# geometryxyz/mental-poker

Measured on AMD Instinct MI355X. Metric: shuffle proofs/sec (prove+verify), higher is better.
Workload: dtype u32 limbs (256-bit Montgomery: 9x29-bit lazy base field, 8x32 scalar field); 1 GPU; pairs: 52-card deck, m=2 n=26, stark curve, shuffle_and_remask + verify_shuffle; rccl_world=1, fixed_base_window_bits=21, unit_counted=prove+verify pairs, streams=1, aggregate_keys=1, transcript_lanes=1, prover_streams=1, pipeline_depth=0, validated_once=False, full=False

## Files before the change

mental-poker_amd/csrc/engine_core.hpp:

```cpp
#pragma once
#include "engine_base.hpp"
#include "kernels_bucket.hpp"
#include "kernels_decompress.hpp"
#include "kernels_sigma.hpp"
#include "kernels_open.hpp"
#include "kernels_deal.hpp"
#include "serialize_host.hpp"
#include "setup_host.hpp"

namespace mp {

static const uint32_t FCHUNK = 8;
static const uint32_t VCHUNK = 64;
static const uint32_t NORM_CHUNK = 64;
static const uint32_t BUCKET_MIN = 2048;
static const uint32_t BUCKET_MIN_SMALL_BATCH = 512;

struct PhaseDev {
  DevBuf<Term> recode, tables, fterms, vterms, cterms, cterms2, cterms0;
  DevBuf<Job> fjobs, vjobs, cjobs, cjobs2, cjobs0;
  DevBuf<BJob> bjobs;
  DevBuf<Term> bterms;
  DevBuf<BTermPos> bpos;
  DevBuf<Job> wcjobs;
// ... 34 lines not shown
    b_bits = ph.b_bits;
    n_recode = (uint32_t)ph.recode.size();
    n_tables = (uint32_t)ph.tables.size();
    n_f = (uint32_t)ph.fjobs.size();
    n_v = (uint32_t)ph.vjobs.size();
    n_c = (uint32_t)ph.cjobs.size();
    n_tslots = ph.n_tslots;
    n_dslots = ph.n_dslots;
    normalize = ph.normalize;
  }
};

struct Workspace {
  uint32_t fw = 8;
  uint32_t Bpad = 0;
  uint32_t nS = 0, nP = 0, nJ = 0, nD = 0, nT = 0, nwin = 0, stage_words = 0;
  DevBuf<uint32_t> S, P, J, T, NS, NS2, stage, seed, direct;
  DevBuf<uint32_t> W;
  DevBuf<int8_t> D;
  DevBuf<int16_t> D16;
  uint32_t d8_bytes = 0;
  DevBuf<uint32_t> bk_sorted, bk_park, bk_counter, bk_timing, bk_quarters;
  DevBuf<uint16_t> bk_offs;
  void ensure_bucket(uint32_t nslots, uint32_t kpad_max, uint32_t bits, uint32_t xw, rt::Stream s) {
    bk_sorted.alloc((size_t)nslots * kpad_max, s, false);
    bk_park.alloc((size_t)nslots * bk_buckets(bits) * xw, s, false);
    bk_counter.alloc(8, s);
  }
  DevBuf<int32_t> status;
  uint32_t cap = 0;
  void ensure(uint32_t B, uint32_t nS_, uint32_t nP_, uint32_t nJ_, uint32_t nD_, uint32_t nT_, uint32_t nwin_,
              uint32_t stage_words_, rt::Stream s, uint32_t d8_bytes_ = 0) {
    const uint32_t need = (B + 63u) & ~63u;
    const bool grow = !(need <= cap && nS_ <= nS && nP_ <= nP && nJ_ <= nJ && nD_ <= nD && nT_ <= nT && stage_words_ <= stage_words &&
                        d8_bytes_ <= d8_bytes);
    if (grow) {
      cap = std::max(cap, need);
      nS = std::max(nS, nS_); nP = std::max(nP, nP_); nJ = std::max(nJ, nJ_); nD = std::max(nD, nD_); nT = std::max(nT, nT_);
      nwin = nwin_;
      stage_words = std::max(stage_words, stage_words_);
      S.n = P.n = J.n = T.n = NS.n = stage.n = seed.n = direct.n = 0;
      D.n = 0;
      D16.n = 0;
      d8_bytes = std::max(d8_bytes, d8_bytes_);
      D16.alloc((size_t)std::max(d8_bytes, 4u) * cap, s);
      status.n = 0;
      S.alloc((size_t)nS * cap * 8, s);
      P.alloc((size_t)nP * cap * 2 * fw, s);
      J.alloc((size_t)nJ * cap * 3 * fw, s);
      D.alloc((size_t)std::max(nD, 1u) * nwin * cap, s);
      T.alloc((size_t)std::max(nT, 1u) * VB_ENTRIES * cap * 2 * fw, s);
      size_t norm_max = std::max((size_t)nT * 8, (size_t)nJ) * cap;
      NS.alloc(norm_max * fw, s);
      stage.alloc((size_t)stage_words * cap, s);
      seed.alloc((size_t)8 * cap, s);
      direct.alloc((size_t)2 * cap, s);
      status.alloc(cap, s);
      Bpad = need;
      return;
    }
    if (Bpad != need) {
      Bpad = need;
      rt::dzero(J.p, (size_t)nJ * Bpad * 3 * fw * sizeof(uint32_t), s);
    }
  }
};

template <class C>
struct Table : mp_table {
// ... 202 lines not shown
  DevBuf<uint32_t> vflag;
  uint32_t* flag_word(bool vlane, rt::Stream s) {
    if (!vflag.n) vflag.alloc(2, s);
    rt::dzero(vflag.p + (vlane ? 1 : 0), 4, s);
    return vflag.p + (vlane ? 1 : 0);
  }
  bool read_flag(bool vlane) {
    uint32_t flag = 0;
    rt::d2h(&flag, vflag.p + (vlane ? 1 : 0), 4, ctx->stream);
    rt::stream_sync(ctx->stream);
    return flag != 0;
  }
  uint32_t nwin = 0;
  FbGeom fbg{8, 32, 255};
  uint32_t init_seed[8];
  DevBuf<uint8_t> io_a, io_b, io_c, io_d, io_e, io_f;
  DevBuf<int32_t> io_status;

  static bool wire_point_host(const uint8_t* p, Aff<C>& out) {
    alignas(8) uint8_t tmp[G_::PB];
    memcpy(tmp, p, G_::PB);
    return wire_to_aff<C>(tmp, out);
  }

  void build_plans(PlanSet* set, bool keyed) {
    rt::Stream s = ctx->stream;
    for (int k = 0; k < N_PLANS; ++k) {
      PlanSet& q = set[k];
      const PlanParams& pp = pprm[k];
      const uint32_t bmin = (bucket_min && k == 3) ? std::min(bucket_min, BUCKET_MIN_SMALL_BATCH) : bucket_min;
// ... 76 lines not shown
      fe_pack<F>(bases[i].x, &flat[i * G_::PW]);
      fe_pack<F>(bases[i].y, &flat[i * G_::PW + G_::FW]);
    }
    fbpts.upload(flat, s);
    build_fixed_tables(fb.count());

    build_plans(ps, false);
    {
      Blake2sState st;
      blake2s_init(st);
      uint32_t mblk[16] = {0};
      memcpy(mblk, "Shuffle Proof", 13);
      blake2s_compress(st, mblk, 13, true);
      memcpy(init_seed, st.h, 32);
    }
    rt::stream_sync(s);
    return MP_OK;
  }

  void normalize_flat(const uint32_t* src, uint32_t* dst, uint32_t* scratch, size_t count) {
    if (!count) return;
    const uint32_t ch = cur_norm_chunk;
    NormArgs a{src, dst, scratch, (uint32_t)count, (uint32_t)((count + ch - 1) / ch), ch};
    MP_RUN(k_normalize, C, a.nthreads, 1, a);
  }

  void build_narrow_tables(const uint32_t* pts, uint32_t nb, const FbGeom& gh, uint32_t h2, uint32_t* out) {
    rt::Stream s = ctx->stream;
    DevBuf<uint32_t> WJ, W, EJ, scratch;
    const size_t nwinpts = (size_t)nb * gh.windows, nent = nwinpts * gh.entries;
// ... 62 lines not shown
      const uint32_t kc = (uint32_t)std::min(slice, K - k0);
      build_narrow_tables(pts.p + k0 * G_::PW, kc, g8, 8u, ks.FB.p + k0 * per_key);
    }
    rt::stream_sync(s);
    return MP_OK;
  }
  DevBuf<uint32_t> ks_keys_main, ks_keys_vlane;
  const uint8_t* gather_keys(uint32_t B, const mp_keyset* ks, const uint32_t* kidx, int32_t* status, bool vlane = false) {
    DevBuf<uint32_t>& ks_keys = vlane ? ks_keys_vlane : ks_keys_main;
    ks_keys.alloc((size_t)B * (G_::PB / 4), ctx->stream, false);
    GatherKeysArgs ga{ks->wire.p, kidx, ks_keys.p, status, (uint32_t)ks->K};
    MP_RUN(k_gather_keys, C, B, G_::PB / 4, ga);
    return reinterpret_cast<const uint8_t*>(ks_keys.p);
  }

  uint32_t stage_words_needed() const {
    const size_t tb = G_::PB + 1;
    size_t bytes = (size_t)(3 + n + 1 + 4 * N) * tb + 16 + 32;
    bytes = std::max(bytes, (size_t)(1 + 6 * m) * tb + 32);
    return (uint32_t)(bytes / 4 + 4);
  }

  void reserve(size_t B) override { reserve_for(B, false); }
  void reserve_for(size_t B, bool keyed) { reserve_ws(ws, B, keyed); }
  void reserve_ws(Workspace& ws, size_t B, bool keyed) {
    if (keyed) ensure_keyed();
    PlanSet& q = pick((uint32_t)B, keyed);
    uint32_t nS = std::max(q.pplan.lay.nS, q.vplan.lay.nS), nP = std::max(q.pplan.lay.nP, q.vplan.lay.nP);
    uint32_t nJ = std::max(q.pplan.nJ, q.vplan.nJ), nD = std::max(q.vph.n_dslots, q.vmph.n_dslots),
             nT = std::max(q.vph.n_tslots, q.vmph.n_tslots);
    uint32_t d8 = std::max(q.vph.b_dig_bytes, q.vmph.b_dig_bytes);
    for (int i = 0; i < 6; ++i) {
      nD = std::max(nD, q.pph[i].n_dslots);
      nT = std::max(nT, q.pph[i].n_tslots);
      d8 = std::max(d8, q.pph[i].b_dig_bytes);
    }
    if (keyed) {
      nD = std::max(nD, key_d_first + N);
      nT = std::max(nT, key_t_first + nwin);
    }
    ws.fw = G_::FW;
    ws.ensure((uint32_t)B, nS, nP, nJ, nD, nT, nwin, stage_words_needed(), ctx->stream, d8);
    if (&ws == &this->ws && overlap_max && B <= overlap_max) ws.NS2.alloc((size_t)m * ws.Bpad * G_::FW, ctx->stream, false);
  }

  enum : uint32_t { PH_RECODE = 1, PH_TABLES = 2, PH_MSM = 4, PH_NORM = 8, PH_ALL = 15 };
  void run_phase(PhaseDev& ph, Workspace& w, uint32_t B, uint32_t parts = PH_ALL, uint32_t norm_only = NO_SLOT, uint32_t norm_skip = NO_SLOT,
                 uint32_t* scratch = nullptr) {
    if (!scratch) scratch = w.NS.p;
    if (parts & PH_TABLES) run_tables(ph, w, B, scratch);
    if (parts & PH_RECODE) run_recode(ph, w, B);
    if (parts & PH_MSM) run_msms(ph, w, B);
    if (parts & PH_NORM) run_normalize(ph, w, B, norm_only, norm_skip, scratch);
  }
#ifdef MP_EXP_QUAD_MAX
  uint32_t quad_max_lanes = MP_EXP_QUAD_MAX;
#else
// ... 204 lines not shown
    }
  }

  FsStatementArgs statement_args(Workspace& w, uint32_t p_deck, uint32_t p_shuf, uint32_t p_cA, uint32_t s_x, uint32_t p_pk = NO_SLOT) {
    FsStatementArgs a{};
    a.f = FsDev{w.stage.p, w.seed.p, w.Bpad};
    a.S = w.S.p;
    a.P = w.P.p;
    a.fbpts = fbpts.p;
    memcpy(a.init_seed, init_seed, 32);
    a.m = m; a.n = n; a.N = N;
    a.p_deck = p_deck; a.p_shuf = p_shuf; a.p_cA = p_cA; a.s_x = s_x;
    a.p_pk = p_pk;
    a.W = nullptr;
    a.w_deck = a.w_shuf = NO_SLOT;
    return a;
  }
  FsqGeom fsq_geom(uint32_t B) const {
    uint32_t lpp = 64;
    while (lpp > 4 && (uint64_t)B * lpp > 65536u) lpp >>= 1;
    return FsqGeom{lpp, B};
  }
  static uint32_t fsq_waves(const FsqGeom& g) { return (g.B + 64u / g.lpp - 1) / (64u / g.lpp); }
  bool fs_quad(uint32_t B) const { return fs_lanes == 4 || (fs_lanes == 0 && B <= FSQ_MAX_BATCH); }
  void run_fs_round1(const FsStatementArgs& a, uint32_t B) {
    if (fs_quad(B)) {
      FsqStatementArgs q{a, fsq_geom(B)};
      MP_WAVE_RUN(k_fsq_round1, C, fsq_waves(q.g), 0, q);
    } else {
      MP_RUN(k_fs_round1, C, B, 1, a);
    }
  }
  void run_fs_round(const FsRoundArgs& a, uint32_t B) {
    if (fs_quad(B)) {
      FsqRoundArgs q{a, fsq_geom(B)};
      MP_WAVE_RUN(k_fsq_round, C, fsq_waves(q.g), 0, q);
    } else {
      MP_RUN(k_fs_round, C, B, 1, a);
    }
  }
  void run_verify_fs(const VerifyFsArgs& a, uint32_t B) {
    if (fs_quad(B)) {
      FsqVerifyArgs q{a, fsq_geom(B)};
      MP_WAVE_RUN(k_fsq_verify, C, fsq_waves(q.g), 0, q);
    } else {
      MP_RUN(k_verify_fs, C, B, 1, a);
    }
  }
  uint32_t* wire_words(Workspace& w, uint32_t B, uint32_t decks) {
    const int plan = plan_of(B);
    if (plan != 1 && plan != 3 && plan != 5) return nullptr;
    w.W.alloc((size_t)decks * 2 * N * (G_::PB / 4) * w.Bpad, ctx->stream, false);
    return w.W.p;
  }

  void prove_init(const ProveInitArgs& ia, uint32_t B) {
    if (B <= PROVE_INIT_WAVE_MAX)
// ... 628 lines not shown
            if (j == 0) var(ChainTerm{l.mvar + l.deck + i, g, 1, NO_SLOT, G}, l.deck + i, g);
            else if (j < L) var(ChainTerm{l.mvar + l.deck + i, j * G + g, 1, l.mvar + l.shuf + i, G}, l.deck + i, j * G + g);
            else var(ChainTerm{l.mvar + l.shuf + i, (L - 1) * G + g, 1, NO_SLOT, G}, l.shuf + i, (L - 1) * G + g);
          }
      for (uint32_t j = 0; j < L * G; ++j)
        for (uint32_t slot = l.cA; slot < l.pk; ++slot) var(ChainTerm{l.mvar + slot, j, 1, NO_SLOT, 1}, slot, j);
      if (keyed)
        for (uint32_t g = 0; g < G; ++g) var(ChainTerm{l.mvar + l.pk, g, L, NO_SLOT, G}, l.pk, g);
    });
    chain.dtile_src.upload(chain.tile_src, ctx->stream);
  }
  size_t chain_lane_bytes(uint32_t, bool keyed) override {
    if (keyed) ensure_keyed();
    const VerifyLay& l = (keyed ? psk : ps)[0].vplan.lay;
    const size_t fwb = (size_t)G_::FW * 4, nJ = 4 + bk_windows(R::BITS, 8);
    return (size_t)l.nS * 32 + (size_t)l.nP * 2 * fwb + nJ * 3 * fwb + nwin + (size_t)VB_ENTRIES * 2 * fwb + nJ * fwb + (size_t)stage_words_needed() * 4 + 32 + 8 + 4 + 8;
  }
  size_t chain_lanes_held() const override { return cws.cap; }
  uint32_t chain_group_size(size_t T, uint32_t L, bool keyed) const override { return T < 0x7FFFFFFFu ? chain_group_of((uint32_t)T, L, keyed) : 1u; }
  void size_equations(const ChainPlan& p, uint32_t T, uint32_t L) {
    const uint32_t Tpad = (T + 63u) & ~63u;
    chain_cw.alloc((size_t)L * Tpad * 8, ctx->stream, false);
    chain_cs.alloc((size_t)(p.K + p.nfix) * Tpad * 8, ctx->stream);
    chain_d8.alloc((size_t)p.dev.b_dig_bytes * Tpad, ctx->stream);
  }
  struct EquationArgs {
    uint32_t T, L;
    bool vlane;
    const char* too_many;
    uint32_t pk, G;
    uint32_t* flag;
// ... 28 lines not shown
      gbad[e.vlane ? 1 : 0].alloc(T, s, false);
      gb = gbad[e.vlane ? 1 : 0].p;
    }
    ChainVerdictArgs va{w.J.p, w.direct.p, w.status.p, e.flag ? e.flag : flag_word(e.vlane, s), gb, w.Bpad, T, e.L, 0u, w.P.p, e.pk, e.G, e.status, nullptr};
    run_chain_verdict(va);
  }
  void verify_chain_dev(size_t T_, uint32_t L, const uint8_t* decks, const uint8_t* proofs, int32_t* status, const uint8_t* keys) override {
    const uint32_t T = (uint32_t)T_, B = T * L;
    const bool keyed = keys != nullptr;
    const uint32_t G = chain_group_of(T, L, keyed), Tq = T / G, Lq = L * G;
    build_chain_plan(L, keyed, G);
    PlanSet& q = (keyed ? psk : ps)[0];
    const VerifyLay& l = q.vplan.lay;
    Workspace& w = cws;
    w.fw = G_::FW;
    w.ensure(B, l.nS, l.nP, std::max(chain.nJ, 8u), 0, 0, nwin, stage_words_needed(), ctx->stream, 0);
    const VArgs cv{B, decks, decks + (size_t)T * 2 * N * G_::PB, proofs, status, keys, nullptr, nullptr};
    load_verify_inputs(w, q, cv, false, false);
    run_transcripts(w, q, B, keyed, true, false);
    run_verify_scalars(w, q, B, true);
    size_equations(chain, Tq, Lq);
    run_chain_weights(w, (Tq + 63u) & ~63u, Tq, Lq);
    const EquationArgs e{Tq, Lq, false, "chain verification: too many tables for one launch", keyed ? l.pk : NO_SLOT, G, nullptr, nullptr, status};
    run_equations(w, chain, e, true, [&](uint32_t* run) {
      ChainTileArgs ta{w.P.p, run, chain.dtile_src.p, w.Bpad, Tq, chain.K};
      if ((uint64_t)Tq * chain.K >= ((uint64_t)1 << 32)) throw std::runtime_error("chain verification: too many tables for one launch");
      MP_RUN(k_chain_tile, C, Tq * chain.K, 1, ta);
    });
    if (!read_flag(false)) return;
    refine_groups(cv, gbad[0].p, false, Tq, Lq, false, false, 0, 0, false);
  }
// ... 68 lines not shown
      for (uint32_t j = 0; j < L; ++j)
        for (uint32_t slot = 0; slot < per; ++slot)
          term(ChainTerm{l.mvar + slot, j, 1, NO_SLOT, 1}, bk_tile ? j * per + slot : (slot | (j << 20)));
    });
    return *fresh;
  }
  void verify_group_pass(const VArgs& v, uint32_t L, bool vlane, uint32_t* host_flag, uint32_t* gbad_out) {
    const uint32_t B = v.B, T = B / L;
    const bool keyed = v.keys != nullptr || v.kset != nullptr;
    ChainPlan& gplan = build_group_plan(L, keyed);
    PlanSet& q = (keyed ? psk : ps)[0];
    const VerifyLay& l = q.vplan.lay;
    rt::Stream s = ctx->stream;
    Workspace& w = vlane ? gws : ws;
    w.fw = G_::FW;
    w.ensure(B, l.nS, l.nP, std::max(gplan.nJ, 8u), 0, 0, nwin, stage_words_needed(), s, 0);
    load_verify_inputs(w, q, v, vlane, false);
    run_transcripts(w, q, B, keyed, true, false);
    size_equations(gplan, T, L);
    {
      SideGuard wguard{ctx, false};
      {
        SideFork on_side(ctx);
        run_chain_weights(w, (T + 63u) & ~63u, T, L);
        rt::event_record(ctx->ev_tab, ctx->side);
      }
      run_verify_scalars(w, q, B, true);
      rt::stream_wait(s, ctx->ev_tab);
      wguard.joined = true;
    }
    const uint32_t per = l.pk + (keyed ? 1u : 0u);
// ... 149 lines not shown
          pb.end();
        }
        pb.normalize(l.A, nb);
      } else {
        for (uint32_t i = 0; i < nb; ++i) {
          pb.begin(l.chk + i);
          pb.var(l.z, l.g + i);
          pb.var(l.negc, l.a + i);
          pb.var(l.minus_one, l.A + i);
          pb.end();
        }
      }
    }
    ad.dev.upload(ad.ph, s);
    ad.w.fw = G_::FW;
    ad.w.ensure(B, 6, 3 * nb, next_partial, ad.ph.n_dslots, ad.ph.n_tslots, nwin, (3 * nb * (G_::PB + 1) + 32) / 4 + 4, s);
    Workspace& w = ad.w;
    DevBuf<uint8_t> dg, da, dx, dfs, dseed, dpf;
    DevBuf<int32_t> dst;
    dg.alloc((size_t)B * nb * G_::PB, s, false); da.alloc((size_t)B * nb * G_::PB, s, false); dfs.alloc((size_t)B * 32, s, false);
    dpf.alloc((size_t)B * psz, s, false);
    rt::h2d(dg.p, bases, (size_t)B * nb * G_::PB, s);
    rt::h2d(da.p, publics, (size_t)B * nb * G_::PB, s);
    rt::h2d(dfs.p, fs_init, (size_t)B * 32, s);
    rt::dzero(w.status.p, (size_t)w.Bpad * 4, s);
    LoadPointsArgs lg{dg.p, w.P.p, w.status.p, w.Bpad, nb, l.g};
    MP_RUN(k_load_points, C, B, nb, lg);
    LoadPointsArgs la{da.p, w.P.p, w.status.p, w.Bpad, nb, l.a};
    MP_RUN(k_load_points, C, B, nb, la);
    check_subgroup(w, B, l.g, 2 * nb);
    const FsDev f{w.stage.p, w.seed.p, w.Bpad};
// ... 82 lines not shown
        op.nD = std::max(op.nD, ph->n_dslots);
        op.nT = std::max(op.nT, ph->n_tslots);
      }
      op.vdev.upload(op.vph, s);
      op.rdev1.upload(op.rph1, s);
      op.rdev2.upload(op.rph2, s);
      Blake2sState st;
      blake2s_init(st);
      uint32_t mblk[16] = {0};
      memcpy(mblk, "Reveal Proof", 12);
      blake2s_compress(st, mblk, 12, true);
      memcpy(op.fs_seed, st.h, 32);
      op.ready = true;
    }
    op.w.fw = G_::FW;
    op.w.ensure(B, 6, 6, op.nJ, op.nD, op.nT, nwin, (6 * (G_::PB + 1) + 32) / 4 + 4, s);
    op.fs.alloc((size_t)op.w.cap * 32, s, false);
    rt::dzero(op.w.status.p, (size_t)op.w.Bpad * 4, s);
  }
  OpenStmtArgs open_stmt_args(size_t K, const uint8_t* keys, const uint8_t* cards, uint32_t T, const uint32_t* signer) {
    OpenStmtArgs a{};
    Workspace& w = op.w;
    a.P = w.P.p; a.S = w.S.p; a.status = w.status.p;
    a.keys = keys; a.cards = cards; a.signer = signer;
    a.fbpts = fbpts.p;
    a.fs_init = op.fs.p;
    memcpy(a.fs_seed, op.fs_seed, 32);
    a.l = make_sigma_lay(2);
    a.Bpad = w.Bpad; a.K = (uint32_t)K; a.T = T; a.g_base = FixedBases{n}.G();
    return a;
  }
// ... 190 lines not shown
      deal.pdev1.upload(deal.pph1, s);
      deal.pdev2.upload(deal.pph2, s);
      deal.sdev.upload(deal.sph, s);
      const char* names[2] = {"Masking Proof", "Remasking Proof"};
      for (int k = 0; k < 2; ++k) {
        Blake2sState st;
        blake2s_init(st);
        uint32_t mblk[16] = {0};
        memcpy(mblk, names[k], strlen(names[k]));
        blake2s_compress(st, mblk, (uint32_t)strlen(names[k]), true);
        memcpy(deal.fs_seed[k], st.h, 32);
      }
      deal.ready = true;
    }
    deal.w.fw = G_::FW;
    deal.w.ensure(B, 6, d.nP, deal.nJ, deal.nD, deal.nT, nwin, (6 * (G_::PB + 1) + 32) / 4 + 4, s);
    deal.fs.alloc((size_t)deal.w.cap * 32, s, false);
    rt::dzero(deal.w.status.p, (size_t)deal.w.Bpad * 4, s);
  }
  DealStmtArgs deal_stmt_args(int kind, size_t K, const uint8_t* keys, const uint32_t* key_index, const uint8_t* inputs) {
    DealStmtArgs a{};
    Workspace& w = deal.w;
    a.P = w.P.p; a.J = w.J.p; a.S = w.S.p; a.status = w.status.p;
    a.keys = keys; a.key_index = key_index; a.inputs = inputs;
    a.fbpts = fbpts.p;
    a.fs_init = deal.fs.p;
    memcpy(a.fs_seed, deal.fs_seed[kind == MP_DEAL_REMASK ? 1 : 0], 32);
    a.l = make_deal_lay();
    a.Bpad = w.Bpad; a.K = (uint32_t)K; a.g_base = FixedBases{n}.G(); a.remask = kind == MP_DEAL_REMASK ? 1u : 0u;
    return a;
  }
// ... 281 lines not shown
```

mental-poker_amd/csrc/hash.hpp:

```cpp
#pragma once
#include <cstdint>

#include "field.hpp"

namespace mp {

MP_HD uint32_t rotr32(uint32_t x, int c) { return (x >> c) | (x << (32 - c)); }
MP_HD uint32_t rotl32(uint32_t x, int c) { return (x << c) | (x >> (32 - c)); }

struct Blake2sState {
  uint32_t h[8];
};

MP_HD void blake2s_init(Blake2sState& s) {
  const uint32_t iv[8] = {0x6A09E667u, 0xBB67AE85u, 0x3C6EF372u, 0xA54FF53Au, 0x510E527Fu, 0x9B05688Cu, 0x1F83D9ABu, 0x5BE0CD19u};
#pragma unroll
  for (int i = 0; i < 8; ++i) s.h[i] = iv[i];
  s.h[0] ^= 0x01010020u;
}

#define MP_B2S_G(a, b, c, d, x, y) \
  v[a] = v[a] + v[b] + (x);        \
  v[d] = rotr32(v[d] ^ v[a], 16);  \
  v[c] = v[c] + v[d];              \
// ... 66 lines not shown
  w.acc |= (uint64_t)x << (8 * w.nb);
  w.base[(size_t)w.widx * w.stride] = (uint32_t)w.acc;
  w.widx++;
  w.acc >>= 32;
}
MP_HD void stage_byte(StageWriter& w, uint32_t x) {
  w.acc |= (uint64_t)(x & 0xFFu) << (8 * w.nb);
  w.nb++;
  if (w.nb == 4) {
    w.base[(size_t)w.widx * w.stride] = (uint32_t)w.acc;
    w.widx++;
    w.acc = 0;
    w.nb = 0;
  }
}
MP_HD uint32_t stage_len(const StageWriter& w) { return w.widx * 4u + w.nb; }

MP_HD void blake2s_staged(StageWriter& w, uint32_t out[8]) {
  const uint32_t len = stage_len(w);
  if (w.nb) w.base[(size_t)w.widx * w.stride] = (uint32_t)w.acc;
  const uint32_t nwords = (len + 3u) / 4u;
  Blake2sState s;
  blake2s_init(s);
  uint32_t nblocks = (len + 63u) / 64u;
  if (nblocks == 0) nblocks = 1;
  for (uint32_t blk = 0; blk < nblocks; ++blk) {
    uint32_t m[16];
#pragma unroll
    for (int i = 0; i < 16; ++i) {
      uint32_t wi = blk * 16u + i;
      m[i] = wi < nwords ? w.base[(size_t)wi * w.stride] : 0u;
    }
    const bool last = blk + 1 == nblocks;
    const uint64_t t = last ? (uint64_t)len : (uint64_t)(blk + 1) * 64u;
    blake2s_compress(s, m, t, last);
  }
#pragma unroll
  for (int i = 0; i < 8; ++i) out[i] = s.h[i];
}

struct B2sBlock {
  uint32_t w[16];
};
struct B2sSeed {
  uint32_t s[8];
};
MP_HD uint32_t sel4(uint32_t j, uint32_t w0, uint32_t w1, uint32_t w2, uint32_t w3) {
  const uint32_t lo = (j & 1u) ? w1 : w0, hi = (j & 1u) ? w3 : w2;
  return (j & 2u) ? hi : lo;
}
#define MP_B2Q_HALF(x, y)                                                             \
  wv.lanes([&](uint32_t l) {                                                          \
    const uint32_t j = l & 3u;                                                        \
// ... 164 lines not shown
```

mental-poker_amd/csrc/kernels_proto.hpp:

```cpp
#pragma once
#include "hash.hpp"
#include "kernels_msm.hpp"

namespace mp {

enum : int32_t { ST_OK = 0, ST_BAD_ENCODING = -1, ST_BAD_PERMUTATION = -2 };

MP_HD void status_fail(int32_t* status, uint32_t b, int32_t code) {
  status[b] = code;
}

template <class F>
MP_HD bool wire_to_fe(const uint8_t* p, Fe<F>& out) {
  uint32_t k[F::NW];
  const uint32_t* q = reinterpret_cast<const uint32_t*>(p);
#pragma unroll
  for (int i = 0; i < F::NW; ++i) k[i] = q[i];
  const bool ok = fe_canonical_in_range<F>(k);
  out = fe_from_canonical<F>(k);
  return ok;
}
template <class F>
MP_HD void fe_to_wire(const Fe<F>& a, uint8_t* p) {
  uint32_t k[F::NW];
// ... 234 lines not shown
  wv.lanes([&](uint32_t lane) {
    if (lane != 0) return;
    st_fe<R>(a.S + s_off(l.zt + l.m + 1, a.Bpad, b), fe_zero<R>());
    st_fe<R>(a.S + s_off(l.meb + l.m, a.Bpad, b), fe_zero<R>());
    st_fe<R>(a.S + s_off(l.mes + l.m, a.Bpad, b), fe_zero<R>());
    st_fe<R>(a.S + s_off(l.svdelta + l.n - 1, a.Bpad, b), fe_zero<R>());
  });
}
MP_WAVE_KERNEL(k_prove_init_w, ProveInitArgs, body_prove_init_w)

struct FsDev {
  uint32_t* stage;
  uint32_t* seed;
  uint32_t Bpad;
};
template <class C>
MP_HD void fs_put_point(StageWriter& w, const Aff<C>& p) {
  typedef typename C::FqP F;
  constexpr int FW = F::NW;
  uint32_t k[FW];
  if (aff_is_inf<C>(p)) {
    for (int i = 0; i < FW; ++i) stage_word(w, 0);
    stage_word(w, 1);
    for (int i = 1; i < FW; ++i) stage_word(w, 0);
    stage_byte(w, 1);
    return;
  }
  fe_to_canonical<F>(p.x, k);
#pragma unroll
  for (int i = 0; i < FW; ++i) stage_word(w, k[i]);
  fe_to_canonical<F>(p.y, k);
#pragma unroll
  for (int i = 0; i < FW; ++i) stage_word(w, k[i]);
  stage_byte(w, 0);
}
template <class C>
MP_HD void fs_put_wire_point(StageWriter& w, const uint32_t* W, uint32_t slot, uint32_t Bpad, uint32_t b) {
  constexpr int FW = C::FqP::NW, WW = 2 * FW;
  uint32_t k[WW], nz = 0;
  ld_words<WW>(W + ((size_t)slot * Bpad + b) * WW, k);
#pragma unroll
  for (int i = 0; i < WW; ++i) nz |= k[i];
  if (nz == 0) {
    for (int i = 0; i < FW; ++i) stage_word(w, 0);
    stage_word(w, 1);
    for (int i = 1; i < FW; ++i) stage_word(w, 0);
    stage_byte(w, 1);
    return;
  }
#pragma unroll
  for (int i = 0; i < WW; ++i) stage_word(w, k[i]);
  stage_byte(w, 0);
}
MP_HD void fs_load_seed(const FsDev& f, uint32_t b, uint32_t seed[8]) {
#pragma unroll
  for (int i = 0; i < 8; ++i) seed[i] = f.seed[(size_t)i * f.Bpad + b];
}
MP_HD void fs_store_seed(const FsDev& f, uint32_t b, const uint32_t seed[8]) {
#pragma unroll
  for (int i = 0; i < 8; ++i) f.seed[(size_t)i * f.Bpad + b] = seed[i];
}
MP_HD void fs_finish_absorb(StageWriter& w, uint32_t seed[8]) {
#pragma unroll
  for (int i = 0; i < 8; ++i) stage_word(w, seed[i]);
  blake2s_staged(w, seed);
}
template <class C>
MP_HD void fs_absorb_points(const FsDev& f, const uint32_t* P, uint32_t b, uint32_t seed[8], uint32_t first, uint32_t count) {
  StageWriter w = stage_begin(f.stage, f.Bpad, b);
  for (uint32_t i = 0; i < count; ++i) fs_put_point<C>(w, ld_aff<C>(P + p_off<C>(first + i, f.Bpad, b)));
  fs_finish_absorb(w, seed);
}
template <class C>
MP_HD void fs_challenges(const uint32_t seed[8], uint32_t* S, uint32_t Bpad, uint32_t b, uint32_t slot0, uint32_t slot1) {
  typedef typename C::FrP R;
  FrStream st;
  frstream_init(st, seed);
  st_fe<R>(S + s_off(slot0, Bpad, b), frstream_next<R>(st));
  if (slot1 != NO_SLOT) st_fe<R>(S + s_off(slot1, Bpad, b), frstream_next<R>(st));
}

struct FsStatementArgs {
  FsDev f;
  uint32_t* S;
  const uint32_t* P;
  const uint32_t* fbpts;
  uint32_t init_seed[8];
  uint32_t m, n, N;
  uint32_t p_deck, p_shuf, p_cA, s_x;
  uint32_t p_pk;
  const uint32_t* W;
  uint32_t w_deck, w_shuf;
};
MP_HD uint32_t fs_statement_points(const FsStatementArgs& a) { return 4 + a.n + 4 * a.N; }
template <class C>
MP_HD void fs_put_statement_point(StageWriter& w, const FsStatementArgs& a, uint32_t b, uint32_t i) {
  const FixedBases fb{a.n};
  const uint32_t nfix = 4 + a.n;
  if (i < nfix) {
    if (i == 1 && a.p_pk != NO_SLOT) {
      fs_put_point<C>(w, ld_aff<C>(a.P + p_off<C>(a.p_pk, a.f.Bpad, b)));
      return;
    }
    const uint32_t base = i == 0 ? fb.G() : i == 1 ? fb.pk() : i == 2 ? fb.gen() : i == nfix - 1 ? fb.H() : fb.ck(i - 3);
    fs_put_point<C>(w, ld_aff<C>(a.fbpts + (size_t)base * Geo<C>::PW));
    return;
  }
  i -= nfix;
  const bool second = i >= 2 * a.N;
  if (second) i -= 2 * a.N;
  const uint32_t wslot = second ? a.w_shuf : a.w_deck;
  if (a.W && wslot != NO_SLOT)
    fs_put_wire_point<C>(w, a.W, wslot + i, a.f.Bpad, b);
  else
    fs_put_point<C>(w, ld_aff<C>(a.P + p_off<C>((second ? a.p_shuf : a.p_deck) + i, a.f.Bpad, b)));
}
template <class C>
MP_HD void fs_statement_and_x(const FsStatementArgs& a, uint32_t b, uint32_t seed[8]) {
#pragma unroll
  for (int i = 0; i < 8; ++i) seed[i] = a.init_seed[i];
  StageWriter w = stage_begin(a.f.stage, a.f.Bpad, b);
  const uint32_t npts = fs_statement_points(a);
  for (uint32_t i = 0; i < npts; ++i) fs_put_statement_point<C>(w, a, b, i);
  stage_word(w, a.m); stage_word(w, 0); stage_word(w, a.n); stage_word(w, 0);
  fs_finish_absorb(w, seed);
  fs_absorb_points<C>(a.f, a.P, b, seed, a.p_cA, a.m);
  fs_challenges<C>(seed, a.S, a.f.Bpad, b, a.s_x, NO_SLOT);
}
template <class C>
MP_HD void body_fs_round1(const FsStatementArgs& a, uint32_t b, uint32_t y) {
  uint32_t seed[8];
  fs_statement_and_x<C>(a, b, seed);
  fs_store_seed(a.f, b, seed);
}
MP_KERNEL(k_fs_round1, FsStatementArgs, body_fs_round1)

struct FsStep {
  uint32_t first, count;
  uint32_t first2, count2;
  uint32_t slot0, slot1;
};
struct FsRoundArgs {
  FsDev f;
  uint32_t* S;
  uint32_t* P;
  FsStep step[4];
  uint32_t nsteps;
  uint32_t copy_from, copy_to;
};
template <class C>
MP_HD void fs_run_steps(const FsRoundArgs& a, uint32_t b, uint32_t seed[8]) {
  for (uint32_t s = 0; s < a.nsteps; ++s) {
    const FsStep st = a.step[s];
    StageWriter w = stage_begin(a.f.stage, a.f.Bpad, b);
    for (uint32_t i = 0; i < st.count; ++i) fs_put_point<C>(w, ld_aff<C>(a.P + p_off<C>(st.first + i, a.f.Bpad, b)));
    for (uint32_t i = 0; i < st.count2; ++i) fs_put_point<C>(w, ld_aff<C>(a.P + p_off<C>(st.first2 + i, a.f.Bpad, b)));
    fs_finish_absorb(w, seed);
    if (st.slot0 != NO_SLOT) fs_challenges<C>(seed, a.S, a.f.Bpad, b, st.slot0, st.slot1);
  }
}
template <class C>
MP_HD void body_fs_round(const FsRoundArgs& a, uint32_t b, uint32_t y) {
  if (a.copy_from != NO_SLOT)
    st_aff<C>(a.P + p_off<C>(a.copy_to, a.f.Bpad, b), ld_aff<C>(a.P + p_off<C>(a.copy_from, a.f.Bpad, b)));
  uint32_t seed[8];
  fs_load_seed(a.f, b, seed);
  fs_run_steps<C>(a, b, seed);
  fs_store_seed(a.f, b, seed);
}
MP_KERNEL(k_fs_round, FsRoundArgs, body_fs_round)

struct ProveScalArgs {
// ... 318 lines not shown
  uint32_t* S = a.st.S;
  const uint32_t* P = a.st.P;
  fs_absorb_points<C>(f, P, b, seed, l.cB, m);
  fs_challenges<C>(seed, S, f.Bpad, b, l.y, l.z);
  fs_absorb_points<C>(f, P, b, seed, l.cb, 1);
  fs_absorb_points<C>(f, P, b, seed, l.hB, m);
  fs_challenges<C>(seed, S, f.Bpad, b, l.hx, l.hy);
  fs_absorb_points<C>(f, P, b, seed, l.zcA0, 2 + 2 * m + 1);
  fs_challenges<C>(seed, S, f.Bpad, b, l.zx, NO_SLOT);
  fs_absorb_points<C>(f, P, b, seed, l.svcd, 3);
  fs_challenges<C>(seed, S, f.Bpad, b, l.svx, NO_SLOT);
  fs_absorb_points<C>(f, P, b, seed, l.mecA0, 1 + 2 * m + 4 * m);
  fs_challenges<C>(seed, S, f.Bpad, b, l.mx, NO_SLOT);
  if (a.merge) {
    typedef typename C::FrP R;
    StageWriter w = stage_begin(f.stage, f.Bpad, b);
    for (uint32_t i = 0; i < 5 * l.n + 9; ++i) {
      uint32_t k[8];
      fe_to_canonical<R>(ld_fe<R>(S + s_off(l.zabar + i, f.Bpad, b)), k);
#pragma unroll
      for (int t = 0; t < 8; ++t) stage_word(w, k[t]);
    }
    fs_finish_absorb(w, seed);
    FrStream st;
    frstream_init(st, seed);
    for (uint32_t k = 0; k < (uint32_t)VC_COUNT; ++k) st_fe<R>(S + s_off(l.mr + k, f.Bpad, b), frstream_next<R>(st));
#pragma unroll
    for (int t = 0; t < 8; ++t) f.seed[(size_t)t * f.Bpad + b] = seed[t];
  }
}
MP_KERNEL(k_verify_fs, VerifyFsArgs, body_verify_fs)

struct FsqGeom {
  uint32_t lpp, B;
};
struct FsqLane {
// ... 529 lines not shown
```

mental-poker_amd/csrc/kernels_sigma.hpp:

```cpp
#pragma once
#include "kernels_proto.hpp"

namespace mp {

struct SigmaLay {
  uint32_t nb;
  uint32_t x, r, c, z, negc, minus_one;
  uint32_t g, a, A, chk;
};
MP_HD SigmaLay make_sigma_lay(uint32_t nb) {
  SigmaLay l;
  l.nb = nb;
  l.x = 0; l.r = 1; l.c = 2; l.z = 3; l.negc = 4; l.minus_one = 5;
  l.g = 0; l.a = nb; l.A = 2 * nb; l.chk = 3 * nb;
  return l;
}

struct SigmaInitArgs {
  uint32_t* S;
  const uint8_t* seeds;
  SigmaLay l;
  uint32_t Bpad;
  FsDev f;
  const uint32_t* P;
  const uint8_t* fs_init;
};
template <class C>
MP_HD void body_sigma_init(const SigmaInitArgs& a, uint32_t b, uint32_t y) {
  typedef typename C::FrP R;
  uint32_t key[8];
  const uint32_t* sw = reinterpret_cast<const uint32_t*>(a.seeds + (size_t)b * 32);
#pragma unroll
  for (int i = 0; i < 8; ++i) key[i] = sw[i];
  {
    StageWriter w = stage_begin(a.f.stage, a.f.Bpad, b);
    uint32_t k[8];
    fe_to_canonical<R>(ld_fe<R>(a.S + s_off(a.l.x, a.Bpad, b)), k);
#pragma unroll
    for (int i = 0; i < 8; ++i) stage_word(w, k[i]);
    const uint32_t* fw = reinterpret_cast<const uint32_t*>(a.fs_init + (size_t)b * 32);
#pragma unroll
    for (int i = 0; i < 8; ++i) stage_word(w, fw[i]);
    fs_finish_absorb(w, key);
  }
  fs_absorb_points<C>(a.f, a.P, b, key, a.l.g, 2 * a.l.nb);
  FrStream st;
  frstream_init(st, key);
  st_fe<R>(a.S + s_off(a.l.r, a.Bpad, b), frstream_next<R>(st));
}
MP_KERNEL(k_sigma_init, SigmaInitArgs, body_sigma_init)

struct SigmaFsArgs {
  FsDev f;
  uint32_t* S;
  const uint32_t* P;
  const uint8_t* fs_init;
  SigmaLay l;
// ... 81 lines not shown
```

Before: 709,700 proofs/s.

## Stream Fiat-Shamir transcript hashing through shared memory and precompute fixed-base prefix

Replaces the staged transcript path, which wrote every message word to a global-memory stage buffer and then re-read it to hash, with an incremental BLAKE2s writer. The writer buffers one 64-byte block per thread in shared memory and compresses as blocks fill. The hash state over the fixed statement points (generators, key, bases, H) is computed once on the host and resumed per lane, so those points are not re-absorbed in every proof. The per-lane stage buffer is now allocated only for the four-lanes-per-hash path. The cost is 16 KB of shared memory per block, which may lower occupancy, and a non-inlined compress call.

```diff
diff --git a/mental-poker_amd/csrc/engine_core.hpp b/mental-poker_amd/csrc/engine_core.hpp
--- a/mental-poker_amd/csrc/engine_core.hpp
+++ b/mental-poker_amd/csrc/engine_core.hpp
@@ -72,7 +72,7 @@
 struct Workspace {
   uint32_t fw = 8;
   uint32_t Bpad = 0;
-  uint32_t nS = 0, nP = 0, nJ = 0, nD = 0, nT = 0, nwin = 0, stage_words = 0;
+  uint32_t nS = 0, nP = 0, nJ = 0, nD = 0, nT = 0, nwin = 0, stage_words = 0, stage_cap = 0;
   DevBuf<uint32_t> S, P, J, T, NS, NS2, stage, seed, direct;
   DevBuf<uint32_t> W;
   DevBuf<int8_t> D;
@@ -90,14 +90,17 @@
   void ensure(uint32_t B, uint32_t nS_, uint32_t nP_, uint32_t nJ_, uint32_t nD_, uint32_t nT_, uint32_t nwin_,
               uint32_t stage_words_, rt::Stream s, uint32_t d8_bytes_ = 0) {
     const uint32_t need = (B + 63u) & ~63u;
-    const bool grow = !(need <= cap && nS_ <= nS && nP_ <= nP && nJ_ <= nJ && nD_ <= nD && nT_ <= nT && stage_words_ <= stage_words &&
-                        d8_bytes_ <= d8_bytes);
+    if (stage_words_ && (stage_words_ > stage_words || need > stage_cap)) {
+      stage_words = std::max(stage_words, stage_words_);
+      stage_cap = std::max(stage_cap, need);
+      stage.alloc((size_t)stage_words * stage_cap, s);
+    }
+    const bool grow = !(need <= cap && nS_ <= nS && nP_ <= nP && nJ_ <= nJ && nD_ <= nD && nT_ <= nT && d8_bytes_ <= d8_bytes);
     if (grow) {
       cap = std::max(cap, need);
       nS = std::max(nS, nS_); nP = std::max(nP, nP_); nJ = std::max(nJ, nJ_); nD = std::max(nD, nD_); nT = std::max(nT, nT_);
       nwin = nwin_;
-      stage_words = std::max(stage_words, stage_words_);
-      S.n = P.n = J.n = T.n = NS.n = stage.n = seed.n = direct.n = 0;
+      S.n = P.n = J.n = T.n = NS.n = seed.n = direct.n = 0;
       D.n = 0;
       D16.n = 0;
       d8_bytes = std::max(d8_bytes, d8_bytes_);
@@ -110,7 +113,6 @@
       T.alloc((size_t)std::max(nT, 1u) * VB_ENTRIES * cap * 2 * fw, s);
       size_t norm_max = std::max((size_t)nT * 8, (size_t)nJ) * cap;
       NS.alloc(norm_max * fw, s);
-      stage.alloc((size_t)stage_words * cap, s);
       seed.alloc((size_t)8 * cap, s);
       direct.alloc((size_t)2 * cap, s);
       status.alloc(cap, s);
@@ -343,6 +345,7 @@
   uint32_t nwin = 0;
   FbGeom fbg{8, 32, 255};
   uint32_t init_seed[8];
+  StreamPrefix fs_prefix;
   DevBuf<uint8_t> io_a, io_b, io_c, io_d, io_e, io_f;
   DevBuf<int32_t> io_status;
 
@@ -449,6 +452,15 @@
       blake2s_compress(st, mblk, 13, true);
       memcpy(init_seed, st.h, 32);
     }
+    {
+      StreamWriter w = stream_begin();
+      fs_put_point<C>(w, G);
+      fs_put_point<C>(w, pkp);
+      fs_put_point<C>(w, gen);
+      for (uint32_t j = 0; j < n; ++j) fs_put_point<C>(w, bases[fb.ck(j)]);
+      fs_put_point<C>(w, H);
+      fs_prefix = stream_export(w);
+    }
     rt::stream_sync(s);
     return MP_OK;
   }
@@ -541,7 +553,8 @@
     return reinterpret_cast<const uint8_t*>(ks_keys.p);
   }
 
-  uint32_t stage_words_needed() const {
+  uint32_t stage_words_needed(uint32_t B) const {
+    if (!fs_quad(B)) return 0;
     const size_t tb = G_::PB + 1;
     size_t bytes = (size_t)(3 + n + 1 + 4 * N) * tb + 16 + 32;
     bytes = std::max(bytes, (size_t)(1 + 6 * m) * tb + 32);
@@ -567,7 +580,7 @@
       nT = std::max(nT, key_t_first + nwin);
     }
     ws.fw = G_::FW;
-    ws.ensure((uint32_t)B, nS, nP, nJ, nD, nT, nwin, stage_words_needed(), ctx->stream, d8);
+    ws.ensure((uint32_t)B, nS, nP, nJ, nD, nT, nwin, stage_words_needed((uint32_t)B), ctx->stream, d8);
     if (&ws == &this->ws && overlap_max && B <= overlap_max) ws.NS2.alloc((size_t)m * ws.Bpad * G_::FW, ctx->stream, false);
   }
 
@@ -802,6 +815,7 @@
     a.p_pk = p_pk;
     a.W = nullptr;
     a.w_deck = a.w_shuf = NO_SLOT;
+    a.pre = fs_prefix;
     return a;
   }
   FsqGeom fsq_geom(uint32_t B) const {
@@ -811,8 +825,12 @@
   }
   static uint32_t fsq_waves(const FsqGeom& g) { return (g.B + 64u / g.lpp - 1) / (64u / g.lpp); }
   bool fs_quad(uint32_t B) const { return fs_lanes == 4 || (fs_lanes == 0 && B <= FSQ_MAX_BATCH); }
+  static void need_stage(const FsDev& f) {
+    if (!f.stage) throw std::runtime_error("transcript: this batch runs four lanes per hash and its workspace holds no message stage");
+  }
   void run_fs_round1(const FsStatementArgs& a, uint32_t B) {
     if (fs_quad(B)) {
+      need_stage(a.f);
       FsqStatementArgs q{a, fsq_geom(B)};
       MP_WAVE_RUN(k_fsq_round1, C, fsq_waves(q.g), 0, q);
     } else {
@@ -821,6 +839,7 @@
   }
   void run_fs_round(const FsRoundArgs& a, uint32_t B) {
     if (fs_quad(B)) {
+      need_stage(a.f);
       FsqRoundArgs q{a, fsq_geom(B)};
       MP_WAVE_RUN(k_fsq_round, C, fsq_waves(q.g), 0, q);
     } else {
@@ -829,6 +848,7 @@
   }
   void run_verify_fs(const VerifyFsArgs& a, uint32_t B) {
     if (fs_quad(B)) {
+      need_stage(a.st.f);
       FsqVerifyArgs q{a, fsq_geom(B)};
       MP_WAVE_RUN(k_fsq_verify, C, fsq_waves(q.g), 0, q);
     } else {
@@ -1487,7 +1507,7 @@
     if (keyed) ensure_keyed();
     const VerifyLay& l = (keyed ? psk : ps)[0].vplan.lay;
     const size_t fwb = (size_t)G_::FW * 4, nJ = 4 + bk_windows(R::BITS, 8);
-    return (size_t)l.nS * 32 + (size_t)l.nP * 2 * fwb + nJ * 3 * fwb + nwin + (size_t)VB_ENTRIES * 2 * fwb + nJ * fwb + (size_t)stage_words_needed() * 4 + 32 + 8 + 4 + 8;
+    return (size_t)l.nS * 32 + (size_t)l.nP * 2 * fwb + nJ * 3 * fwb + nwin + (size_t)VB_ENTRIES * 2 * fwb + nJ * fwb + (size_t)stage_words_needed(1) * 4 + 32 + 8 + 4 + 8;
   }
   size_t chain_lanes_held() const override { return cws.cap; }
   uint32_t chain_group_size(size_t T, uint32_t L, bool keyed) const override { return T < 0x7FFFFFFFu ? chain_group_of((uint32_t)T, L, keyed) : 1u; }
@@ -1546,7 +1566,7 @@
     const VerifyLay& l = q.vplan.lay;
     Workspace& w = cws;
     w.fw = G_::FW;
-    w.ensure(B, l.nS, l.nP, std::max(chain.nJ, 8u), 0, 0, nwin, stage_words_needed(), ctx->stream, 0);
+    w.ensure(B, l.nS, l.nP, std::max(chain.nJ, 8u), 0, 0, nwin, stage_words_needed(B), ctx->stream, 0);
     const VArgs cv{B, decks, decks + (size_t)T * 2 * N * G_::PB, proofs, status, keys, nullptr, nullptr};
     load_verify_inputs(w, q, cv, false, false);
     run_transcripts(w, q, B, keyed, true, false);
@@ -1645,7 +1665,7 @@
     rt::Stream s = ctx->stream;
     Workspace& w = vlane ? gws : ws;
     w.fw = G_::FW;
-    w.ensure(B, l.nS, l.nP, std::max(gplan.nJ, 8u), 0, 0, nwin, stage_words_needed(), s, 0);
+    w.ensure(B, l.nS, l.nP, std::max(gplan.nJ, 8u), 0, 0, nwin, stage_words_needed(B), s, 0);
     load_verify_inputs(w, q, v, vlane, false);
     run_transcripts(w, q, B, keyed, true, false);
     size_equations(gplan, T, L);
@@ -1825,7 +1845,7 @@
     }
     ad.dev.upload(ad.ph, s);
     ad.w.fw = G_::FW;
-    ad.w.ensure(B, 6, 3 * nb, next_partial, ad.ph.n_dslots, ad.ph.n_tslots, nwin, (3 * nb * (G_::PB + 1) + 32) / 4 + 4, s);
+    ad.w.ensure(B, 6, 3 * nb, next_partial, ad.ph.n_dslots, ad.ph.n_tslots, nwin, 0, s);
     Workspace& w = ad.w;
     DevBuf<uint8_t> dg, da, dx, dfs, dseed, dpf;
     DevBuf<int32_t> dst;
@@ -1938,7 +1958,7 @@
       op.ready = true;
     }
     op.w.fw = G_::FW;
-    op.w.ensure(B, 6, 6, op.nJ, op.nD, op.nT, nwin, (6 * (G_::PB + 1) + 32) / 4 + 4, s);
+    op.w.ensure(B, 6, 6, op.nJ, op.nD, op.nT, nwin, 0, s);
     op.fs.alloc((size_t)op.w.cap * 32, s, false);
     rt::dzero(op.w.status.p, (size_t)op.w.Bpad * 4, s);
   }
@@ -2159,7 +2179,7 @@
       deal.ready = true;
     }
     deal.w.fw = G_::FW;
-    deal.w.ensure(B, 6, d.nP, deal.nJ, deal.nD, deal.nT, nwin, (6 * (G_::PB + 1) + 32) / 4 + 4, s);
+    deal.w.ensure(B, 6, d.nP, deal.nJ, deal.nD, deal.nT, nwin, 0, s);
     deal.fs.alloc((size_t)deal.w.cap * 32, s, false);
     rt::dzero(deal.w.status.p, (size_t)deal.w.Bpad * 4, s);
   }
diff --git a/mental-poker_amd/csrc/hash.hpp b/mental-poker_amd/csrc/hash.hpp
--- a/mental-poker_amd/csrc/hash.hpp
+++ b/mental-poker_amd/csrc/hash.hpp
@@ -104,29 +104,146 @@
     w.nb = 0;
   }
 }
-MP_HD uint32_t stage_len(const StageWriter& w) { return w.widx * 4u + w.nb; }
-
-MP_HD void blake2s_staged(StageWriter& w, uint32_t out[8]) {
-  const uint32_t len = stage_len(w);
-  if (w.nb) w.base[(size_t)w.widx * w.stride] = (uint32_t)w.acc;
-  const uint32_t nwords = (len + 3u) / 4u;
+struct StreamWriter {
   Blake2sState s;
-  blake2s_init(s);
-  uint32_t nblocks = (len + 63u) / 64u;
-  if (nblocks == 0) nblocks = 1;
-  for (uint32_t blk = 0; blk < nblocks; ++blk) {
-    uint32_t m[16];
-#pragma unroll
-    for (int i = 0; i < 16; ++i) {
-      uint32_t wi = blk * 16u + i;
-      m[i] = wi < nwords ? w.base[(size_t)wi * w.stride] : 0u;
-    }
-    const bool last = blk + 1 == nblocks;
-    const uint64_t t = last ? (uint64_t)len : (uint64_t)(blk + 1) * 64u;
-    blake2s_compress(s, m, t, last);
-  }
-#pragma unroll
-  for (int i = 0; i < 8; ++i) out[i] = s.h[i];
+  uint32_t t;
+  uint32_t widx;
+  uint64_t acc;
+  uint32_t nb;
+#if !defined(__HIP_DEVICE_COMPILE__)
+  uint32_t blk[16];
+#endif
+};
+#if defined(__HIP_DEVICE_COMPILE__)
+__device__ __forceinline__ uint32_t* stream_col() {
+  __shared__ uint32_t mp_stream_blocks[16 * 256];
+  return mp_stream_blocks + threadIdx.x;
+}
+#define MP_STREAM_SLOT(w, i) (stream_col()[(i) * 256u])
+__device__ __noinline__ Blake2sState stream_compress_col(Blake2sState s, uint32_t t, uint32_t last) {
+  const uint32_t* col = stream_col();
+  uint32_t m[16];
+#pragma unroll
+  for (int i = 0; i < 16; ++i) m[i] = col[i * 256];
+  blake2s_compress(s, m, (uint64_t)t, last != 0);
+  return s;
+}
+#else
+#define MP_STREAM_SLOT(w, i) ((w).blk[i])
+#endif
+MP_HD void stream_compress(StreamWriter& w, uint32_t t, bool last) {
+#if defined(__HIP_DEVICE_COMPILE__)
+  w.s = stream_compress_col(w.s, t, last ? 1u : 0u);
+#else
+  blake2s_compress(w.s, w.blk, (uint64_t)t, last);
+#endif
+}
+MP_HD StreamWriter stream_begin() {
+  StreamWriter w;
+  blake2s_init(w.s);
+  w.t = 0;
+  w.widx = 0;
+  w.acc = 0;
+  w.nb = 0;
+  return w;
+}
+struct StreamPrefix {
+  uint32_t h[8];
+  uint32_t blk[16];
+  uint32_t t, widx, nb, acc;
+};
+MP_HD StreamPrefix stream_export(StreamWriter& w) {
+  StreamPrefix p;
+#pragma unroll
+  for (int i = 0; i < 8; ++i) p.h[i] = w.s.h[i];
+#pragma unroll
+  for (int i = 0; i < 16; ++i) p.blk[i] = (uint32_t)i < w.widx ? MP_STREAM_SLOT(w, i) : 0u;
+  p.t = w.t;
+  p.widx = w.widx;
+  p.nb = w.nb;
+  p.acc = (uint32_t)w.acc;
+  return p;
+}
+MP_HD StreamWriter stream_resume(const StreamPrefix& p) {
+  StreamWriter w;
+#pragma unroll
+  for (int i = 0; i < 8; ++i) w.s.h[i] = p.h[i];
+  w.t = p.t;
+  w.widx = p.widx;
+  w.acc = p.acc;
+  w.nb = p.nb;
+#pragma unroll
+  for (int i = 0; i < 16; ++i) MP_STREAM_SLOT(w, i) = p.blk[i];
+  return w;
+}
+template <int N>
+MP_HD void stream_words(StreamWriter& w, const uint32_t* k) {
+  static_assert(N >= 1 && N <= 16, "at most one block boundary");
+  uint32_t o[N];
+  const uint32_t sh = 8u * w.nb;
+#pragma unroll
+  for (int i = 0; i < N; ++i) {
+    w.acc |= (uint64_t)k[i] << sh;
+    o[i] = (uint32_t)w.acc;
+    w.acc >>= 32;
+  }
+  const uint32_t room = 16u - w.widx;
+#pragma unroll
+  for (int i = 0; i < N; ++i)
+    if ((uint32_t)i < room) MP_STREAM_SLOT(w, w.widx + i) = o[i];
+  if (room < (uint32_t)N) {
+    w.t += 64u;
+    stream_compress(w, w.t, false);
+#pragma unroll
+    for (int i = 0; i < N; ++i)
+      if ((uint32_t)i >= room) MP_STREAM_SLOT(w, (uint32_t)i - room) = o[i];
+    w.widx = (uint32_t)N - room;
+  } else {
+    w.widx += (uint32_t)N;
+  }
+}
+MP_HD void put_word(StreamWriter& w, uint32_t x) { stream_words<1>(w, &x); }
+MP_HD void put_byte(StreamWriter& w, uint32_t x) {
+  w.acc |= (uint64_t)(x & 0xFFu) << (8 * w.nb);
+  w.nb++;
+  if (w.nb == 4) {
+    const uint32_t x4 = (uint32_t)w.acc;
+    w.acc = 0;
+    w.nb = 0;
+    stream_words<1>(w, &x4);
+  }
+}
+MP_HD uint32_t stream_len(const StreamWriter& w) { return w.t + w.widx * 4u + w.nb; }
+MP_HD void stream_finish(StreamWriter& w, uint32_t out[8]) {
+  const uint32_t len = stream_len(w);
+  if (w.nb) {
+    const uint32_t x = (uint32_t)w.acc;
+    w.acc = 0;
+    w.nb = 0;
+    stream_words<1>(w, &x);
+  }
+#pragma unroll
+  for (int i = 0; i < 16; ++i)
+    if ((uint32_t)i >= w.widx) MP_STREAM_SLOT(w, i) = 0u;
+  stream_compress(w, len, true);
+#pragma unroll
+  for (int i = 0; i < 8; ++i) out[i] = w.s.h[i];
+}
+MP_HD void put_word(StageWriter& w, uint32_t x) { stage_word(w, x); }
+MP_HD void put_byte(StageWriter& w, uint32_t x) { stage_byte(w, x); }
+template <int N>
+MP_HD void put_words(StageWriter& w, const uint32_t* k) {
+#pragma unroll
+  for (int i = 0; i < N; ++i) stage_word(w, k[i]);
+}
+template <int N>
+MP_HD void put_words(StreamWriter& w, const uint32_t* k) {
+  if constexpr (N <= 16) {
+    stream_words<N>(w, k);
+  } else {
+    stream_words<16>(w, k);
+    put_words<N - 16>(w, k + 16);
+  }
 }
 
 struct B2sBlock {
diff --git a/mental-poker_amd/csrc/kernels_proto.hpp b/mental-poker_amd/csrc/kernels_proto.hpp
--- a/mental-poker_amd/csrc/kernels_proto.hpp
+++ b/mental-poker_amd/csrc/kernels_proto.hpp
@@ -272,43 +272,30 @@
   uint32_t* seed;
   uint32_t Bpad;
 };
-template <class C>
-MP_HD void fs_put_point(StageWriter& w, const Aff<C>& p) {
+template <class C, class Wr>
+MP_HD void fs_put_point(Wr& w, const Aff<C>& p) {
   typedef typename C::FqP F;
   constexpr int FW = F::NW;
+  const bool inf = aff_is_inf<C>(p);
   uint32_t k[FW];
-  if (aff_is_inf<C>(p)) {
-    for (int i = 0; i < FW; ++i) stage_word(w, 0);
-    stage_word(w, 1);
-    for (int i = 1; i < FW; ++i) stage_word(w, 0);
-    stage_byte(w, 1);
-    return;
-  }
   fe_to_canonical<F>(p.x, k);
-#pragma unroll
-  for (int i = 0; i < FW; ++i) stage_word(w, k[i]);
+  put_words<FW>(w, k);
   fe_to_canonical<F>(p.y, k);
-#pragma unroll
-  for (int i = 0; i < FW; ++i) stage_word(w, k[i]);
-  stage_byte(w, 0);
-}
-template <class C>
-MP_HD void fs_put_wire_point(StageWriter& w, const uint32_t* W, uint32_t slot, uint32_t Bpad, uint32_t b) {
+  if (inf) k[0] = 1u;
+  put_words<FW>(w, k);
+  put_byte(w, inf ? 1u : 0u);
+}
+template <class C, class Wr>
+MP_HD void fs_put_wire_point(Wr& w, const uint32_t* W, uint32_t slot, uint32_t Bpad, uint32_t b) {
   constexpr int FW = C::FqP::NW, WW = 2 * FW;
   uint32_t k[WW], nz = 0;
   ld_words<WW>(W + ((size_t)slot * Bpad + b) * WW, k);
 #pragma unroll
   for (int i = 0; i < WW; ++i) nz |= k[i];
-  if (nz == 0) {
-    for (int i = 0; i < FW; ++i) stage_word(w, 0);
-    stage_word(w, 1);
-    for (int i = 1; i < FW; ++i) stage_word(w, 0);
-    stage_byte(w, 1);
-    return;
-  }
-#pragma unroll
-  for (int i = 0; i < WW; ++i) stage_word(w, k[i]);
-  stage_byte(w, 0);
+  if (nz == 0) k[FW] = 1u;
+  put_words<FW>(w, k);
+  put_words<FW>(w, k + FW);
+  put_byte(w, nz == 0 ? 1u : 0u);
 }
 MP_HD void fs_load_seed(const FsDev& f, uint32_t b, uint32_t seed[8]) {
 #pragma unroll
@@ -318,15 +305,17 @@
 #pragma unroll
   for (int i = 0; i < 8; ++i) f.seed[(size_t)i * f.Bpad + b] = seed[i];
 }
-MP_HD void fs_finish_absorb(StageWriter& w, uint32_t seed[8]) {
-#pragma unroll
-  for (int i = 0; i < 8; ++i) stage_word(w, seed[i]);
-  blake2s_staged(w, seed);
-}
-template <class C>
-MP_HD void fs_absorb_points(const FsDev& f, const uint32_t* P, uint32_t b, uint32_t seed[8], uint32_t first, uint32_t count) {
-  StageWriter w = stage_begin(f.stage, f.Bpad, b);
-  for (uint32_t i = 0; i < count; ++i) fs_put_point<C>(w, ld_aff<C>(P + p_off<C>(first + i, f.Bpad, b)));
+MP_HD void fs_finish_absorb(StreamWriter& w, uint32_t seed[8]) {
+  put_words<8>(w, seed);
+  stream_finish(w, seed);
+}
+template <class C>
+MP_HD void fs_absorb_points(const FsDev& f, const uint32_t* P, uint32_t b, uint32_t seed[8], uint32_t first, uint32_t count,
+                            uint32_t first2 = 0, uint32_t count2 = 0) {
+  StreamWriter w = stream_begin();
+#pragma unroll 1
+  for (uint32_t i = 0; i < count + count2; ++i)
+    fs_put_point<C>(w, ld_aff<C>(P + p_off<C>(i < count ? first + i : first2 + (i - count), f.Bpad, b)));
   fs_finish_absorb(w, seed);
 }
 template <class C>
@@ -349,10 +338,11 @@
   uint32_t p_pk;
   const uint32_t* W;
   uint32_t w_deck, w_shuf;
+  StreamPrefix pre;
 };
 MP_HD uint32_t fs_statement_points(const FsStatementArgs& a) { return 4 + a.n + 4 * a.N; }
-template <class C>
-MP_HD void fs_put_statement_point(StageWriter& w, const FsStatementArgs& a, uint32_t b, uint32_t i) {
+template <class C, class Wr>
+MP_HD void fs_put_statement_point(Wr& w, const FsStatementArgs& a, uint32_t b, uint32_t i) {
   const FixedBases fb{a.n};
   const uint32_t nfix = 4 + a.n;
   if (i < nfix) {
@@ -377,10 +367,13 @@
 MP_HD void fs_statement_and_x(const FsStatementArgs& a, uint32_t b, uint32_t seed[8]) {
 #pragma unroll
   for (int i = 0; i < 8; ++i) seed[i] = a.init_seed[i];
-  StageWriter w = stage_begin(a.f.stage, a.f.Bpad, b);
+  const bool keyed = a.p_pk != NO_SLOT;
+  StreamWriter w = keyed ? stream_begin() : stream_resume(a.pre);
   const uint32_t npts = fs_statement_points(a);
-  for (uint32_t i = 0; i < npts; ++i) fs_put_statement_point<C>(w, a, b, i);
-  stage_word(w, a.m); stage_word(w, 0); stage_word(w, a.n); stage_word(w, 0);
+#pragma unroll 1
+  for (uint32_t i = keyed ? 0u : 4u + a.n; i < npts; ++i) fs_put_statement_point<C>(w, a, b, i);
+  const uint32_t mn[4] = {a.m, 0u, a.n, 0u};
+  put_words<4>(w, mn);
   fs_finish_absorb(w, seed);
   fs_absorb_points<C>(a.f, a.P, b, seed, a.p_cA, a.m);
   fs_challenges<C>(seed, a.S, a.f.Bpad, b, a.s_x, NO_SLOT);
@@ -410,10 +403,7 @@
 MP_HD void fs_run_steps(const FsRoundArgs& a, uint32_t b, uint32_t seed[8]) {
   for (uint32_t s = 0; s < a.nsteps; ++s) {
     const FsStep st = a.step[s];
-    StageWriter w = stage_begin(a.f.stage, a.f.Bpad, b);
-    for (uint32_t i = 0; i < st.count; ++i) fs_put_point<C>(w, ld_aff<C>(a.P + p_off<C>(st.first + i, a.f.Bpad, b)));
-    for (uint32_t i = 0; i < st.count2; ++i) fs_put_point<C>(w, ld_aff<C>(a.P + p_off<C>(st.first2 + i, a.f.Bpad, b)));
-    fs_finish_absorb(w, seed);
+    fs_absorb_points<C>(a.f, a.P, b, seed, st.first, st.count, st.first2, st.count2);
     if (st.slot0 != NO_SLOT) fs_challenges<C>(seed, a.S, a.f.Bpad, b, st.slot0, st.slot1);
   }
 }
@@ -762,12 +752,12 @@
   fs_challenges<C>(seed, S, f.Bpad, b, l.mx, NO_SLOT);
   if (a.merge) {
     typedef typename C::FrP R;
-    StageWriter w = stage_begin(f.stage, f.Bpad, b);
+    StreamWriter w = stream_begin();
+#pragma unroll 1
     for (uint32_t i = 0; i < 5 * l.n + 9; ++i) {
       uint32_t k[8];
       fe_to_canonical<R>(ld_fe<R>(S + s_off(l.zabar + i, f.Bpad, b)), k);
-#pragma unroll
-      for (int t = 0; t < 8; ++t) stage_word(w, k[t]);
+      put_words<8>(w, k);
     }
     fs_finish_absorb(w, seed);
     FrStream st;
diff --git a/mental-poker_amd/csrc/kernels_sigma.hpp b/mental-poker_amd/csrc/kernels_sigma.hpp
--- a/mental-poker_amd/csrc/kernels_sigma.hpp
+++ b/mental-poker_amd/csrc/kernels_sigma.hpp
@@ -33,14 +33,14 @@
 #pragma unroll
   for (int i = 0; i < 8; ++i) key[i] = sw[i];
   {
-    StageWriter w = stage_begin(a.f.stage, a.f.Bpad, b);
+    StreamWriter w = stream_begin();
     uint32_t k[8];
     fe_to_canonical<R>(ld_fe<R>(a.S + s_off(a.l.x, a.Bpad, b)), k);
-#pragma unroll
-    for (int i = 0; i < 8; ++i) stage_word(w, k[i]);
+    put_words<8>(w, k);
     const uint32_t* fw = reinterpret_cast<const uint32_t*>(a.fs_init + (size_t)b * 32);
 #pragma unroll
-    for (int i = 0; i < 8; ++i) stage_word(w, fw[i]);
+    for (int i = 0; i < 8; ++i) k[i] = fw[i];
+    put_words<8>(w, k);
     fs_finish_absorb(w, key);
   }
   fs_absorb_points<C>(a.f, a.P, b, key, a.l.g, 2 * a.l.nb);
```

New measurement: 713,500 proofs/s (median of 6 runs). No clear change (+0.5%).
